# sebcossu/yocto_raytracing

Measured on AMD Instinct MI355X. Metric: Mrays/sec + ms/frame, instance10000 1920×1080×64spp, 1/2/4/8 MI355X, higher is better.
Workload: dtype f32; 1 GPU; instance10000 1920x1080 8x8 spp, amb 0.1, one frame per step; scene=instance10000, width=1920, height=1080, spp=64, parallelism=single GPU, algorithm=wavefront

## Files before the change

yocto_raytracing_amd/csrc/wavefront.hip:

```cpp
#include <hip/hip_runtime.h>

#include <algorithm>
#include <cstdio>
#include <cstdlib>
#include <cstring>
#include <stdexcept>

#include "packet_trace.h"
#include "trace_common.h"
#include "yrt_render.h"

namespace yrt {
namespace {

constexpr int WF_BLOCK = 256;
#ifndef YRT_PRIMARY_BLOCK
#define YRT_PRIMARY_BLOCK 64
#endif
#ifndef YRT_SHADOW_BLOCK
#define YRT_SHADOW_BLOCK 64
#endif
template <bool PACKET>
constexpr int shadow_block() { return PACKET ? YRT_SHADOW_BLOCK : WF_BLOCK; }
#ifndef YRT_TRACE_WAVES
// ... 41 lines not shown
        const float* rays;
    };
    int capacity;
    int nlevels;
    int need_v;
    int bundles;
    f4* pbox;
    int* lcount;
    int* lskip;
    f4* lists;
    f4* slists;
    int cam_lists;
    int* ccount;
    int* cskip;
    f4* clist;
    unsigned long long* lstats;
};

#ifndef YRT_LEVEL_SEGMENTS
#define YRT_LEVEL_SEGMENTS 8
#endif
constexpr int level_segments = YRT_LEVEL_SEGMENTS;
static_assert(2048 % level_segments == 0, "segment bound (run()) assumes level_segments | 2048");
constexpr int count_stride = 32;
__device__ __forceinline__ int* seg_counter(int* count, int level, int g) {
    return count + (level * level_segments + g) * count_stride;
}

struct chunk_args {
    long long pix0;
    int npix;
    int spp;
    int tiles_x;
};

__device__ __forceinline__ bool pixel_of(const dev_render_args& A, int tiles_x, long long p, int& lx, int& ly,
                                         int& i, int& j) {
    long long t = p / (TILE * TILE);
    int w = (int)(p % (TILE * TILE));
    lx = (int)(t % tiles_x) * TILE + (w % TILE);
    ly = (int)(t / tiles_x) * TILE + (w / TILE);
    if (lx >= A.tile_w || ly >= A.tile_h) return false;
    i = A.x0 + lx;
    int b = ly / A.band, r = ly % A.band;
    j = A.y0 + (b * A.band_stride + A.band_offset) * A.band + r;
    return i < A.width && j < A.height;
}

__device__ __forceinline__ void flush(unsigned long long* counters, int idx, unsigned long long v) {
    unsigned long long s = wave_sum(v);
    if ((threadIdx.x & 63) == 0 && s) atomicAdd(counter_line(counters) + idx, s);
}

template <int N, int BS = WF_BLOCK>
__device__ __forceinline__ void flush_block(unsigned long long* counters, const int (&idx)[N],
                                            const unsigned long long (&v)[N]) {
    __shared__ unsigned long long part[BS / 64][N];
    const int w = threadIdx.x >> 6;
#pragma unroll
    for (int k = 0; k < N; k++) {
        const unsigned long long s = wave_sum(v[k]);
        if ((threadIdx.x & 63) == 0) part[w][k] = s;
    }
    __syncthreads();
    if (threadIdx.x < N) {
        unsigned long long t = 0;
#pragma unroll
        for (int q = 0; q < BS / 64; q++) t += part[q][threadIdx.x];
        const unsigned b = (blockIdx.z * gridDim.y + blockIdx.y) * gridDim.x + blockIdx.x;
        if (t) atomicAdd(counters + (size_t)(b % cnt_slots) * cnt_count + idx[threadIdx.x], t);
    }
}

__device__ __forceinline__ void flush_work(unsigned long long* counters, const work_counts& wc) {
    flush(counters, cnt_box_tests, wc.box);
    flush(counters, cnt_inst_entries, wc.inst);
    flush(counters, cnt_prim_tests, wc.prim);
    flush(counters, cnt_shaded_hits, wc.hits);
    flush(counters, cnt_tex_lookups, wc.tex);
    flush(counters, cnt_wave_node_visits, wc.wnode);
    flush(counters, cnt_wave_prim_visits, wc.wprim);
}

typedef float gvec4 __attribute__((ext_vector_type(4)));
#ifndef YRT_NT_STREAMS
#define YRT_NT_STREAMS 1
#endif
#ifndef YRT_R5_VCONST
#define YRT_R5_VCONST 1
#endif
template <int IMM>
__device__ __forceinline__ float vconst() {
    if (!YRT_R5_VCONST) return __int_as_float(IMM);
    float r;
    asm volatile("v_mov_b32 %0, %1" : "=v"(r) : "n"(IMM));
    return r;
}
__device__ __forceinline__ void gstore(f4* p, int idx, float x, float y, float z, float w) {
    auto* q = (__attribute__((address_space(1))) gvec4*)p + idx;
    if (YRT_NT_STREAMS)
        __builtin_nontemporal_store(gvec4{x, y, z, w}, q);
    else
        *q = gvec4{x, y, z, w};
}
__device__ __forceinline__ void gstore(float* p, int idx, float x) {
    auto* q = (__attribute__((address_space(1))) float*)p + idx;
    if (YRT_NT_STREAMS)
        __builtin_nontemporal_store(x, q);
    else
        *q = x;
}
__device__ __forceinline__ float4 ld4s(const f4* p) {
    if (YRT_NT_STREAMS) {
        const gvec4 v = __builtin_nontemporal_load((const __attribute__((address_space(1))) gvec4*)p);
        return make_float4(v.x, v.y, v.z, v.w);
    }
    return ld4(p);
}
__device__ __forceinline__ float lds1(const float* p) {
    if (YRT_NT_STREAMS) return __builtin_nontemporal_load((const __attribute__((address_space(1))) float*)p);
    return *p;
}
__device__ __forceinline__ unsigned char ldb(const unsigned char* p) {
    if (YRT_NT_STREAMS) return __builtin_nontemporal_load((const __attribute__((address_space(1))) unsigned char*)p);
// ... 1255 lines not shown
        elo = lo, ehi = hi;
    }
    const unsigned long long km = ballot(keep);
    if (keep) {
        f4* out = B.clist + ((size_t)t * camera_list_max + __popcll(km & below)) * 2;
        out[0] = {elo.x, elo.y, elo.z, elo.w};
        out[1] = {ehi.x, ehi.y, ehi.z, ehi.w};
    }
    nf = __popcll(km);
    nskip = (int)wave_sum((unsigned long long)nskip);
    if (lane == 0) B.ccount[t] = nf, B.cskip[t] = nskip;
    YRT_LT_STAMP(lt3);
    YRT_LT_WRITE(0, t, lt1 - lt0, lt2 - lt1, lt3 - lt2, (unsigned long long)nrounds << 32 | (unsigned)nf);
}

__global__ __launch_bounds__(256) void k_list_stats(wf_buffers B, int ntiles, int nlists) {
    __shared__ unsigned long long part[list_sums][256 / 64];
    unsigned long long v[list_sums] = {};
    const int stride = gridDim.x * 256;
    if (B.cam_lists)
        for (int i = blockIdx.x * 256 + (int)threadIdx.x; i < ntiles; i += stride) {
            const int n = B.ccount[i];
            v[0] += n < 0 ? camera_list_max + 1 : n, v[1]++, v[4] += (unsigned)B.cskip[i];
        }
    if (B.bundles)
        for (int i = blockIdx.x * 256 + (int)threadIdx.x; i < nlists; i += stride) {
            const int n = B.lcount[i];
            v[2] += n < 0 ? bundle_max + 1 : n, v[3]++, v[5] += (unsigned)B.lskip[i];
        }
    for (int q = 0; q < list_sums; q++) {
        const unsigned long long t = wave_sum(v[q]);
        if ((threadIdx.x & 63) == 0) part[q][threadIdx.x >> 6] = t;
    }
    __syncthreads();
    if (threadIdx.x < list_sums) {
        const unsigned long long t = part[threadIdx.x][0] + part[threadIdx.x][1] + part[threadIdx.x][2] + part[threadIdx.x][3];
        if (t) atomicAdd(B.lstats + threadIdx.x, t);
    }
}

#ifndef YRT_SHADOW_PERSIST_MIN_ITEMS
#define YRT_SHADOW_PERSIST_MIN_ITEMS 262144
#endif
#ifndef YRT_SHADOW_ITEM_LIGHTS
#define YRT_SHADOW_ITEM_LIGHTS 1
#endif
#ifndef YRT_SHADOW_ITEM_RUN
#define YRT_SHADOW_ITEM_RUN 48
#endif
#ifndef YRT_SHADOW_LDS_RECORDS
#define YRT_SHADOW_LDS_RECORDS 85
#endif

template <int LDSN>
__global__ __launch_bounds__(SP_BLOCK, YRT_SHADOW_WAVES) void k_shadow_persist(dev_scene_view S, int nsamp,
                                                                                int nx, wf_buffers B,
                                                                                unsigned long long* counters,
                                                                                float4 cam4) {
    const vec3f cam_o = xyz(cam4);
    constexpr int WPB = SP_BLOCK / 64;
    constexpr unsigned C = (YRT_SHADOW_ITEM_LIGHTS && LDSN == 0) ? YRT_SHADOW_ITEM_RUN : YRT_SHADOW_LIGHT_MINOR;
    __shared__ float4 lds_nodes[LDSN > 0 ? LDSN * 8 : 1];
    if constexpr (LDSN > 0) {
        const int nrec = LDSN * 8;
        const float4* src = reinterpret_cast<const float4*>(S.wnodes);
        for (int i = threadIdx.x; i < nrec; i += SP_BLOCK) lds_nodes[i] = src[i];
        __syncthreads();
    }
    const int nl = S.nlights;
    constexpr bool IL = YRT_SHADOW_ITEM_LIGHTS && LDSN == 0;
    const unsigned n_items = IL ? (unsigned)nx : (unsigned)nx * (unsigned)nl;
    const unsigned lane = threadIdx.x & 63;
    const unsigned xcd = blockIdx.x % 8u;
    unsigned rays = 0;
    unsigned culled_l = 0;
    constexpr unsigned CS = YRT_SHADOW_BLOCK_CHUNK;
    __shared__ chunk_ring ring;
    const unsigned head = head_items<C, CS>(n_items);
    chunk_ring_init<CS>(ring, B.queue + xcd, B.queue + 8, head / 8u);
#ifdef YRT_TAIL_STATS
    const unsigned long long tail_t0 = __builtin_amdgcn_s_memrealtime();
    unsigned tail_items = 0;
#endif
    for (;;) {
        const unsigned q = chunk_ring_next<CS>(ring, B.queue + xcd, lane, B.queue + 8, head / 8u);
        const unsigned it = split_item<C>(q, xcd, n_items, head);
        if (it >= n_items) break;
#ifdef YRT_TAIL_STATS
        tail_items++;
#endif
        const int bx = IL ? (int)it : (int)(it / (unsigned)nl);
        for (int lq = 0; lq < (IL ? nl : 1); lq++) {
        const int li = IL ? lq : (int)(it % (unsigned)nl);
        float4 lrec[6];
        ld_records_at<6>(S.lights, (unsigned)(6 * li), lrec);
        const frame3f lf = {xyz(lrec[0]), xyz(lrec[1]), xyz(lrec[2]), xyz(lrec[3])};
        const vec3f lp0 = xyz(lrec[4]);
        const int idx = bx * 64 + (int)lane;
        bool valid = false;
        int info = -1;
        float r = 1.0f;
        float4 s1 = {0, 0, 0, 0};
        ray3 sr = {{0, 0, 0}, {0, 0, 1}, 0.01f, 1.0f};
        if (idx < nsamp) {
            float4 s0 = IL ? ld4(B.surf0 + idx) : ld4s(B.surf0 + idx);
            if (YRT_SHADOW_CULL && !YRT_HIT16) s1 = IL ? ld4(B.surf1 + idx) : ld4s(B.surf1 + idx);
            info = sample_state(s0);
            if (info >= 0) {
                const vec3f p = YRT_HIT16 ? hit16_surface(S, s0).p : xyz(s0);
                vec3f tp = transform_point(lf, lp0 - p);
                vec3f l;
                normalize_len(tp, l, r);
                sr = {p, l, 0.01f, r - 0.01f};
                valid = true;
            }
        }
        rays += (unsigned)__popcll(ballot(valid));
        const bool zero_term =
            YRT_SHADOW_CULL && !YRT_HIT16 && light_term_zero(info, xyz(s1), sr.o, cam_o, sr.d, r, xyz(lrec[5]));
        const unsigned long long culled = ballot(zero_term);
        culled_l += zero_term ? 1u : 0u;
        const bool all_culled = YRT_SHADOW_CULL && !YRT_HIT16 && culled == ballot(valid);
        bool occ;
        int lc = -1;
        if (YRT_SHADOW_BUNDLES && LDSN == 0 && B.bundles) {
            const int gl = (bx / bundle_g) * nl + li;
            lc = __builtin_amdgcn_readfirstlane(B.lcount[gl]);
        }
        const f4* tbase = S.wnodes;
        uint32_t troot = (uint32_t)S.wtop_root;
        if (lc > 0) {
            tbase = B.lists;
            troot = (uint32_t)(((bx / bundle_g) * nl + li) * bundle_recs * wide_record_bytes);
        }
        occ = all_culled ? true
                         : lc == 0 ? ((culled >> lane) & 1ull) != 0
                                   : packet_occluded_wide2<LDSN, true>(S, sr, valid, lds_nodes, tbase, troot, culled);
        if (valid) stb(B.occl + (size_t)li * B.capacity + idx, occ ? 1 : 0);
        }
    }
#ifdef YRT_TAIL_STATS
    tail_record(1, tail_t0, tail_items);
#endif
    const unsigned long long mine = lane == 0 ? (unsigned long long)rays : 0ull;
    flush_block<2, SP_BLOCK>(counters, {cnt_shadow_rays, cnt_shadow_culled}, {mine, (unsigned long long)culled_l});
}

#ifndef YRT_SHADE_WAVES
#define YRT_SHADE_WAVES 7
#endif
#ifndef YRT_SHADE_LDS_SRGB
#define YRT_SHADE_LDS_SRGB 1
#endif
#ifndef YRT_FOLD_PREFETCH
#define YRT_FOLD_PREFETCH 0
#endif
#ifndef YRT_SHADE_LEVEL_WAVES
#define YRT_SHADE_LEVEL_WAVES 5
#endif
template <bool COUNT, bool FUSE, int SB, bool OCC4, bool RAYS>
__device__ __forceinline__ void shade_samples(dev_scene_view S, dev_render_args A, int level, int nsamp_level0,
                                              int max_depth, wf_buffers B, unsigned long long* counters, chunk_args C,
                                              float4* __restrict__ out) {
    __shared__ float4 fused_rad[FUSE ? SB : 1];
    __shared__ int cmp_count[SB / 64], cmp_base[SB / 64];
    __shared__ float srgb_lds[YRT_SHADE_LDS_SRGB ? 256 : 1];
    const float* lut = YRT_SHADE_LDS_SRGB ? srgb_lds : S.srgb;
    if (YRT_SHADE_LDS_SRGB && S.ntextures > 0) {
        for (int q = (int)threadIdx.x; q < 256; q += SB) srgb_lds[q] = S.srgb[q];
        __syncthreads();
    }
    work_counts wc;
    unsigned long long truncated = 0;
    const vec3f amb = {A.amb[0], A.amb[1], A.amb[2]};
    const vec3f cam_o = {A.cam.ox, A.cam.oy, A.cam.oz};
    const int stride = gridDim.x * SB;
    const int gout = (int)(blockIdx.x % (unsigned)level_segments);
    const int nseg = FUSE ? 1 : level ? level_segments : 1;
    for (int g = 0; g < nseg; g++) {
    const int n = (!FUSE && level) ? *seg_counter(B.count, level, g) : nsamp_level0;
    const int nround = (n + stride - 1) / stride;
    for (int round = 0; round < nround; round++) {
        const int j = round * stride + blockIdx.x * SB + threadIdx.x;
        const int idx = FUSE ? j : g * B.seg + j;
        bool spawn = false;
        vec3f p = {0, 0, 0}, dr = {0, 0, 0}, rec_d = {0, 0, 0}, rec_la = {0, 0, 0};
        int rec_mat = 0;
        if (j < n) {
            float4 s0 = ld4s(B.surf0 + idx);
            uint32_t occ_bits = 0;
            if constexpr (OCC4) {
#pragma unroll
                for (int q = 0; q < 4; q++) {
                    const int lq = q < S.nlights ? q : 0;
                    const uint32_t ob = ldb(B.occl + (size_t)lq * B.capacity + idx);
                    occ_bits |= (q < S.nlights && ob != 0u) ? 1u << q : 0u;
                }
            }
            const int info = sample_state(s0);
            vec3f R = {0, 0, 0};
            bool write_r = info != -2;
            float4 ro4 = (!FUSE && level) ? ld4(B.ray_o(level) + idx) : make_float4(cam_o.x, cam_o.y, cam_o.z, 0.0f);
            if constexpr (RAYS && !FUSE) {
                if (!level) {
                    const vec3f o = ray_origin(B, idx);
                    ro4 = make_float4(o.x, o.y, o.z, 0.0f);
                }
            }
            float4 pd = {0, 0, 0, 0}, pla = {0, 0, 0, 0}, pkr = {0, 0, 0, 0};
            if (YRT_FOLD_PREFETCH && !FUSE && level) {
                const int parent = ibits(ro4.w);
                pd = ld4(B.rec0(level - 1) + parent), pla = ld4(B.rec1(level - 1) + parent);
                pkr = ld4(S.mats + 4 * ibits(pd.w) + 2);
            }
            if (info >= 0) {
                vec3f nrm;
                vec2f uv;
                int mat, kind;
                if (YRT_HIT16) {
                    const surface sf = hit16_surface(S, s0);
                    p = sf.p, nrm = sf.n, uv = sf.uv, mat = sf.mat, kind = sf.kind;
                } else {
                    const float4 s1 = ld4s(B.surf1 + idx);
                    p = xyz(s0), nrm = xyz(s1), uv = {s1.w, (!YRT_SKIP_UNUSED_V || B.need_v) ? lds1(B.surfv + idx) : 0.0f};
                    mat = info_mat(info), kind = info & 3;
                }
                const vec3f ro = xyz(ro4);
                float4 m0, m1, m2, m3;
                {
                    m0 = ld4(S.mats + 4 * mat), m1 = ld4(S.mats + 4 * mat + 1);
                    m2 = ld4(S.mats + 4 * mat + 2), m3 = ld4(S.mats + 4 * mat + 3);
                }
                const vec3f kd0 = xyz(m0), ks0 = xyz(m1), kr = xyz(m2);
                const float ns = m0.w;
                const int kd_txt = ibits(m1.w), ks_txt = ibits(m2.w);
                const bool reflective = ibits(m3.w) & mat_reflective;
                vec3f la = amb * kd0;
                vec3f tkd = {1, 1, 1}, tks = {1, 1, 1};
                if (kd_txt >= 0) {
                    tkd = eval_texture<COUNT>(S, kd_txt, uv, wc, lut);
                    la = la * tkd;
                }
                if (ks_txt >= 0) tks = eval_texture<COUNT>(S, ks_txt, uv, wc, lut);
                vec3f c = {0.0f, 0.0f, 0.0f};
                vec3f v;
                float vlen;
                normalize_len(ro - p, v, vlen);
                for (int li = 0; li < S.nlights; li++) {
                    if (OCC4 ? ((occ_bits >> li) & 1u) != 0u : ldb(B.occl + (size_t)li * B.capacity + idx) != 0) continue;
                    const f4* lr = S.lights + 6 * li;
                    float4 lrec[6];
                    ld_scalar<6>(lr, lrec);
                    frame3f lf = {xyz(lrec[0]), xyz(lrec[1]), xyz(lrec[2]), xyz(lrec[3])};
                    vec3f lp0 = xyz(lrec[4]), ke = xyz(lrec[5]);
                    vec3f tp = transform_point(lf, lp0 - p);
                    vec3f l, h;
                    float r, hlen;
                    normalize_len(tp, l, r);
                    normalize_len(v + l, h, hlen);
                    vec3f kd = kd0, ks = ks0;
                    if (kd_txt >= 0) kd = kd * tkd;
                    if (ks_txt >= 0) ks = ks * tks;
                    const vec3f ker = div3(ke, r * r);
                    vec3f ld = kd * ker;
                    vec3f ls = ks * ker;
                    if (kind == kind_lines) {
                        float prodnl = dot(nrm, l);
                        float prodnh = dot(nrm, h);
                        if (prodnl < 0.0f) prodnl *= -1;
                        if (prodnh < 0.0f) prodnh *= -1;
                        float sinnl = __builtin_sqrtf(1.0f - prodnl);
                        float sinnh = __builtin_sqrtf(1.0f - prodnh);
                        ld = ld * sinnl;
                        ls = ls * spec_pow(sinnh, ns, ls);
                    } else {
                        ld = ld * smax(0.0f, dot(nrm, l));
                        ls = ls * spec_pow(smax(0.0f, dot(nrm, h)), ns, ls);
                    }
                    c = c + (ld + ls);
                }
                if (!reflective) {
                    R = c + la;
                } else if (FUSE || level + 1 >= max_depth || level + 1 >= B.nlevels) {
                    truncated++;
                    vec3f t = {0.0f * kr.x, 0.0f * kr.y, 0.0f * kr.z};
                    R = (c + t) + la;
                } else {
                    spawn = true;
                    dr = (nrm * 2.0f * dot(nrm, v)) - v;
                    rec_d = c;
                    rec_la = la;
                    rec_mat = mat;
                    write_r = false;
                }
                if (COUNT) wc.hits++;
            }
            if (FUSE) {
                fused_rad[threadIdx.x] = make_float4(R.x, R.y, R.z, 1.0f);
            } else if (write_r) {
                vec3f col = R;
                int lev = level, node = idx;
                while (lev > 0) {
                    const bool pre = YRT_FOLD_PREFETCH && lev == level;
                    const int parent = pre ? ibits(ro4.w) : ibits(B.ray_o(lev)[node].w);
                    const float4 d = pre ? pd : ld4(B.rec0(lev - 1) + parent);
                    const float4 la = pre ? pla : ld4(B.rec1(lev - 1) + parent);
                    const float4 kr = pre ? pkr : ld4(S.mats + 4 * ibits(d.w) + 2);
                    vec3f cc = {d.x, d.y, d.z};
                    cc = cc + vec3f{col.x * kr.x, col.y * kr.y, col.z * kr.z};
                    cc = cc + xyz(la);
                    col = cc, node = parent, lev--;
                }
                B.rad[node] = {col.x, col.y, col.z, 1.0f};
            }
        }
        if constexpr (FUSE) continue;
        const unsigned long long mask = __ballot(spawn);
        const int w = threadIdx.x >> 6, lane = threadIdx.x & 63;
        if (spawn) {
            B.rec0(level)[idx] = {rec_d.x, rec_d.y, rec_d.z, __int_as_float(rec_mat)};
            B.rec1(level)[idx] = {rec_la.x, rec_la.y, rec_la.z, 0};
        }
        if (lane == 0) cmp_count[w] = __popcll(mask);
        __syncthreads();
        if (threadIdx.x == 0) {
            int tot = 0;
            for (int q = 0; q < SB / 64; q++) tot += cmp_count[q];
            int acc = tot ? atomicAdd(seg_counter(B.count, level + 1, gout), tot) : 0;
            for (int q = 0; q < SB / 64; q++) cmp_base[q] = acc, acc += cmp_count[q];
        }
        __syncthreads();
        if (spawn) {
            const int slot = gout * B.seg + cmp_base[w] + __popcll(mask & ((1ull << lane) - 1));
            B.ray_o(level + 1)[slot] = {p.x, p.y, p.z, __int_as_float(idx)};
            B.ray_d(level + 1)[slot] = {dr.x, dr.y, dr.z, 0};
        }
    }
    }
    if (FUSE) {
        __syncthreads();
        const int ppb = SB / C.spp;
        for (int t = (int)threadIdx.x; t < 3 * ppb; t += SB) {
            const int px = t / 3, comp = t - 3 * px;
            const int pl = (int)(blockIdx.x * SB / C.spp) + px;
            int lx, ly, i, j;
            const bool valid = pl < C.npix && pixel_of(A, C.tiles_x, C.pix0 + pl, lx, ly, i, j);
            if (pl < C.npix && lx < A.tile_w && ly < A.tile_h) {
                float v = 0.0f;
                if (valid) {
                    const float* r = reinterpret_cast<const float*>(fused_rad + px * C.spp) + comp;
                    float acc = 0.0f;
                    for (int q = 0; q < C.spp; q++) acc = acc + r[4 * q];
                    v = acc / float(C.spp);
                }
                float* o = reinterpret_cast<float*>(out + (size_t)ly * A.out_stride + lx);
                o[comp] = v;
                if (comp == 0) o[3] = valid ? 1.0f : 0.0f;
            }
        }
    }
    flush(counters, cnt_depth_truncated, truncated);
    if (COUNT) flush_work(counters, wc);
}

template <bool COUNT, bool FUSE, int SB = WF_BLOCK, bool OCC4 = false>
__global__ __launch_bounds__(SB, FUSE ? YRT_SHADE_WAVES : YRT_SHADE_LEVEL_WAVES) void k_shade(dev_scene_view S, dev_render_args A, int level, int nsamp_level0,
                                                    int max_depth, wf_buffers B, unsigned long long* counters,
                                                    chunk_args C, float4* __restrict__ out) {
    shade_samples<COUNT, FUSE, SB, OCC4, false>(S, A, level, nsamp_level0, max_depth, B, counters, C, out);
}

template <bool OCC4>
__global__ __launch_bounds__(WF_BLOCK, YRT_SHADE_LEVEL_WAVES) void k_rays_shade(dev_scene_view S, float3 amb3, int level,
                                                                                int nsamp_level0, int max_depth,
                                                                                wf_buffers B,
                                                                                unsigned long long* counters) {
    dev_render_args A = {};
    A.amb[0] = amb3.x, A.amb[1] = amb3.y, A.amb[2] = amb3.z;
    const chunk_args C = {0, nsamp_level0, 1, 1};
    shade_samples<false, false, WF_BLOCK, OCC4, true>(S, A, level, nsamp_level0, max_depth, B, counters, C, nullptr);
}

constexpr int AQ = 8;
__global__ __launch_bounds__(WF_BLOCK) void k_accumulate(dev_render_args A, chunk_args C, wf_buffers B,
                                                         float4* __restrict__ out) {
    __shared__ float4 stage[WF_BLOCK / 64][64 * (AQ + 1)];
    const int w = threadIdx.x >> 6, lane = threadIdx.x & 63;
    const int pl0 = blockIdx.x * WF_BLOCK + w * 64;
    const int np = max(0, min(64, C.npix - pl0));
    float4* S = stage[w];
    const f4* base = B.rad + (size_t)pl0 * C.spp;
    vec4f acc = {0, 0, 0, 0};
    for (int q0 = 0; q0 < C.spp; q0 += AQ) {
        const int qn = min(AQ, C.spp - q0);
        for (int e = lane; e < np * qn; e += 64) {
            const int px = e / qn, q = e % qn;
            S[px * (AQ + 1) + q] = ld4(base + (size_t)px * C.spp + q0 + q);
        }
        __syncthreads();
        if (lane < np)
            for (int q = 0; q < qn; q++) {
                const float4 c = S[lane * (AQ + 1) + q];
                acc = {acc.x + c.x, acc.y + c.y, acc.z + c.z, acc.w + 1.0f};
            }
        __syncthreads();
    }
    if (lane >= np) return;
    const int pl = pl0 + lane;
    int lx, ly, i, j;
    const bool valid = pixel_of(A, C.tiles_x, C.pix0 + pl, lx, ly, i, j);
    if (lx >= A.tile_w || ly >= A.tile_h) return;
    const float d = float(C.spp);
    out[(size_t)ly * A.out_stride + lx] =
        valid ? make_float4(acc.x / d, acc.y / d, acc.z / d, 1.0f) : make_float4(0.0f, 0.0f, 0.0f, 0.0f);
}

constexpr int pass_planes = pass_count + 1;
struct pass_buffers {
    unsigned mask;
    float4* out[pass_planes];
    f4* smp[pass_count];
};

constexpr int shade_pass_waves = 6;
template <bool FUSE, int SB = WF_BLOCK, bool OCC4 = false>
__global__ __launch_bounds__(SB, FUSE ? shade_pass_waves : YRT_SHADE_LEVEL_WAVES) void k_shade_passes(
    dev_scene_view S, dev_render_args A, int level, int nsamp_level0, int max_depth, wf_buffers B, pass_buffers P,
    unsigned long long* counters, chunk_args C) {
    constexpr int ROW = SB + 1;
    __shared__ float fused[FUSE ? pass_planes * 3 * ROW : 1];
    __shared__ int cmp_count[SB / 64], cmp_base[SB / 64];
    __shared__ float srgb_lds[YRT_SHADE_LDS_SRGB ? 256 : 1];
    const float* lut = YRT_SHADE_LDS_SRGB ? srgb_lds : S.srgb;
    if (YRT_SHADE_LDS_SRGB && S.ntextures > 0) {
// ... 353 lines not shown
        if (e != hipSuccess) return e;
        ds.work_bytes = need;
    }
    wf_buffers B = carve(ds.work, cap, spp, ds.nlights, nlevels);
    B.trel = ds.trel;
    B.seg = seg;
    B.need_v = ds.view.ntextures > 0;
    pass_buffers P = {};
    if (passes) {
        P = *passes;
        char* at = (char*)ds.work + workspace_bytes(cap, spp, ds.nlights, nlevels);
        for (int k = 0; k < pass_count && smp_planes; k++)
            if (P.mask >> k & 1) P.smp[k] = (f4*)at, at += align_up(16 * (size_t)pix_per_chunk * spp);
    }
    bool list_stats = false;
    ds.last_camera_lists = ds.last_bundles = false;
    if (!ds.list_stats_host) {
        hipError_t e =
            hipHostMalloc((void**)&ds.list_stats_host, list_sums * sizeof(unsigned long long), hipHostMallocDefault);
        if (e != hipSuccess) return e;
        memset(ds.list_stats_host, 0, list_sums * sizeof(unsigned long long));
    }
    if (!ds.list_stats_ev) {
        hipError_t e = hipEventCreateWithFlags(&ds.list_stats_ev, hipEventDisableTiming);
        if (e != hipSuccess) return e;
    }
    if (nlevels > 1 && !ds.level_count_host) {
        hipError_t e = hipHostMalloc((void**)&ds.level_count_host, sizeof(int) * level_segments * count_stride,
                                     hipHostMallocDefault);
        if (e != hipSuccess) return e;
    }
    if (nlevels > 1 && !ds.level_count_ev) {
        hipError_t e = hipEventCreateWithFlags(&ds.level_count_ev, hipEventDisableTiming);
        if (e != hipSuccess) return e;
    }
    phase_timer& T = ds.timer;
    const bool stage = ds.lds_staging != 0 && !COUNT && PACKET;
    ds.last_lds_staging = 0;
    const float4 cam4 = make_float4(A.cam.ox, A.cam.oy, A.cam.oz, 0.0f);
    const int stride_grid = 2048;
    if (npix_total == 0 && counters) {
        hipError_t e = hipMemsetAsync(counters, 0, (size_t)cnt_slots * cnt_count * sizeof(unsigned long long), stream);
        if (e != hipSuccess) return e;
    }
    for (long long pix0 = 0; pix0 < npix_total; pix0 += pix_per_chunk) {
        chunk_args C = {pix0, (int)std::min<long long>(pix_per_chunk, npix_total - pix0), spp, tiles_x};
        const int nsamp = C.npix * spp;
        const int grid = (nsamp + WF_BLOCK - 1) / WF_BLOCK;
        constexpr int TB = shadow_block<PACKET>();
        const int tgrid = (nsamp + TB - 1) / TB;
        const bool shadow_persist = !COUNT && PACKET && ds.wide_ok && TB == 64 && ds.nlights > 0 &&
                                    ((long long)tgrid * ds.nlights >= YRT_SHADOW_PERSIST_MIN_ITEMS ||
                                     ds.lists_mode == 1 || stage);
        const bool bundles_possible = YRT_SHADOW_BUNDLES && !stage && shadow_persist &&
                                      bundle_lights(ds.nlights) > 0 && ds.view.nwtop >= YRT_BUNDLE_MIN_TOP;
        const bool cam_lists_possible = YRT_CAMERA_LISTS && YRT_PRIMARY_REL && !stage && !COUNT && PACKET && ds.wide_ok &&
                                        ds.view.nwtop >= YRT_BUNDLE_MIN_TOP;
        const bool lists = ds.lists_mode == 1 || (ds.lists_mode == 0 && spp >= YRT_LISTS_MIN_SPP);
        B.cam_lists = cam_lists_possible && lists;
        B.bundles = bundles_possible && lists;
        ds.last_camera_lists |= B.cam_lists != 0, ds.last_bundles |= B.bundles != 0;
        const bool zero_lstats = (B.cam_lists || B.bundles) && !list_stats;
        list_stats |= zero_lstats;
        int t = T.begin(phase_lists, stream);
        {
            const int nrec = (PACKET && pix0 == 0) ? (int)ds.ntnodes * 2 * spine_len : 0;
            const int count_ints = nlevels > 1 ? (int)(count_bytes(nlevels) / sizeof(int)) : 0;
            const int counter_words = pix0 == 0 && counters ? cnt_slots * cnt_count : 0;
            const int work = std::max(std::max(nrec, count_ints), std::max(counter_words, 32));
            const int nb = std::min((work + WF_BLOCK - 1) / WF_BLOCK, 1024);
            hipLaunchKernelGGL(k_chunk_setup, dim3(nb), dim3(WF_BLOCK), 0, stream, nrec ? ds.view.tpair : nullptr,
                               nrec, A.cam.ox, A.cam.oy, A.cam.oz, ds.trel, B.queue,
                               zero_lstats ? B.lstats : nullptr, B.count, count_ints, counters, counter_words);
        }
        if (B.cam_lists) {
            const int nt = C.npix / (TILE * TILE);
            hipLaunchKernelGGL(k_camera_lists, dim3((nt + 3) / 4), dim3(256), 0, stream, ds.view, A, C, B);
        }
        T.end(t, stream);
        t = T.begin(phase_primary, stream);
        bool persist = false;
        if constexpr (!COUNT && PACKET) {
            persist = ((long long)nsamp + 63) / 64 >= (long long)YRT_PRIMARY_PERSIST_MIN_ITEMS;
            if (persist) {
                const int nb = ds.num_cus * (YRT_PRIMARY_WAVES * 4 * 64 / YRT_PRIMARY_SP_BLOCK);
                if (B.cam_lists)
                    hipLaunchKernelGGL((k_primary_persist<SE, 0, true>), dim3(nb), dim3(YRT_PRIMARY_SP_BLOCK), 0,
                                       stream, ds.view, A, C, B, counters);
                else if (stage && YRT_PRIMARY_REL) {
                    hipLaunchKernelGGL((k_primary_persist<SE, YRT_PRIMARY_LDS_RECORDS, false>), dim3(nb),
                                       dim3(YRT_PRIMARY_SP_BLOCK), 0, stream, ds.view, A, C, B, counters);
                    ds.last_lds_staging |= 1;
                } else
                    hipLaunchKernelGGL((k_primary_persist<SE, 0, false>), dim3(nb), dim3(YRT_PRIMARY_SP_BLOCK), 0,
                                       stream, ds.view, A, C, B, counters);
            }
        }
        if (!persist) {
            const dim3 pg((nsamp + YRT_PRIMARY_BLOCK - 1) / YRT_PRIMARY_BLOCK);
            if (B.cam_lists)
                hipLaunchKernelGGL((k_primary<COUNT, PACKET, SE, true>), pg, dim3(YRT_PRIMARY_BLOCK), 0, stream, ds.view,
                                   A, C, B, counters);
            else
                hipLaunchKernelGGL((k_primary<COUNT, PACKET, SE, false>), pg, dim3(YRT_PRIMARY_BLOCK), 0, stream,
                                   ds.view, A, C, B, counters);
        }
        T.end(t, stream);
        for (int level = 0; level < nlevels; level++) {
            if (level > 0) {
                t = T.begin(phase_bounce, stream);
                hipLaunchKernelGGL((k_bounce<COUNT, PACKET, SE>), dim3(stride_grid), dim3(WF_BLOCK), 0, stream, ds.view,
                                   level, B, counters);
                T.end(t, stream);
                hipError_t e = hipEventSynchronize(ds.level_count_ev);
                if (e != hipSuccess) return e;
                bool any = false;
                for (int g = 0; g < level_segments; g++) any |= ds.level_count_host[g * count_stride] != 0;
                if (!any) break;
            }
            if (ds.nlights > 0) {
                dim3 sg(level ? stride_grid * WF_BLOCK / TB : tgrid, ds.nlights);
                if (level == 0 && shadow_persist && B.bundles) {
                    t = T.begin(phase_lists, stream);
                    if (YRT_BUNDLE_FUSED && YRT_BUNDLE_SUPER && bundle_g * super_bundles <= 256) {
                        const long long ns = (long long)super_count(nsamp) * ds.nlights;
                        hipLaunchKernelGGL(k_bundle_lists<true>, dim3((unsigned)ns), dim3(256), 0, stream, ds.view, B,
                                           tgrid);
                    } else {
                        if (YRT_BUNDLE_SUPER) {
                            const long long ns = (long long)super_count(nsamp) * ds.nlights;
                            hipLaunchKernelGGL(k_bundle_super, dim3((unsigned)((ns + 3) / 4)), dim3(256), 0, stream,
                                               ds.view, B, tgrid);
                        }
                        const long long nw = (long long)bundle_count(nsamp) * ds.nlights;
                        hipLaunchKernelGGL(k_bundle_lists<false>, dim3((unsigned)((nw + 3) / 4)), dim3(256), 0, stream,
                                           ds.view, B, tgrid);
                    }
                    T.end(t, stream);
                }
                t = T.begin(phase_shadow, stream);
                if (level == 0 && shadow_persist) {
                    const int nb = ds.num_cus * (YRT_SHADOW_WAVES * 4 * 64 / SP_BLOCK);
                    constexpr int L = YRT_SHADOW_LDS_RECORDS;
                    if (stage && L > 0 && ds.view.nwtop >= L) {
                        hipLaunchKernelGGL((k_shadow_persist<L>), dim3(nb), dim3(SP_BLOCK), 0, stream, ds.view,
                                           nsamp, tgrid, B, counters, cam4);
                        ds.last_lds_staging |= 2;
                    } else
                        hipLaunchKernelGGL((k_shadow_persist<0>), dim3(nb), dim3(SP_BLOCK), 0, stream, ds.view,
                                           nsamp, tgrid, B, counters, cam4);
                } else if (!COUNT && PACKET && ds.wide_ok)
                    hipLaunchKernelGGL((k_shadow<COUNT, PACKET, SE, true>), sg, dim3(TB), 0,
                                       stream, ds.view, level, nsamp, B, counters, cam4);
                else
                    hipLaunchKernelGGL((k_shadow<COUNT, PACKET, SE, false>), sg, dim3(TB), 0,
                                       stream, ds.view, level, nsamp, B, counters, cam4);
                T.end(t, stream);
            }
            t = T.begin(phase_shade, stream);
            const bool occ4 = ds.nlights <= 4;
#define YRT_SHADE_LAUNCH(FU, SBV, GRID)                                                                          \
    do {                                                                                                        \
        if (occ4)                                                                                               \
            hipLaunchKernelGGL((k_shade<COUNT, FU, SBV, true>), GRID, dim3(SBV), 0, stream, ds.view, A, level, nsamp, \
                               A.max_depth, B, counters, C, out);                                               \
        else                                                                                                    \
            hipLaunchKernelGGL((k_shade<COUNT, FU, SBV, false>), GRID, dim3(SBV), 0, stream, ds.view, A, level,      \
                               nsamp, A.max_depth, B, counters, C, out);                                        \
    } while (0)
#define YRT_SHADE_PASSES_LAUNCH(FU, GRID)                                                                          \
    do {                                                                                                          \
        if (occ4)                                                                                                 \
            hipLaunchKernelGGL((k_shade_passes<FU, WF_BLOCK, true>), GRID, dim3(WF_BLOCK), 0, stream, ds.view, A, level, \
                               nsamp, A.max_depth, B, P, counters, C);                                            \
        else                                                                                                      \
            hipLaunchKernelGGL((k_shade_passes<FU, WF_BLOCK, false>), GRID, dim3(WF_BLOCK), 0, stream, ds.view, A,  \
                               level, nsamp, A.max_depth, B, P, counters, C);                                     \
    } while (0)
            if (passes) {
                if constexpr (!COUNT) {
                    if (fuse)
                        YRT_SHADE_PASSES_LAUNCH(true, dim3(grid));
                    else
                        YRT_SHADE_PASSES_LAUNCH(false, dim3(level ? stride_grid : grid));
                }
            } else if (fuse) {
                YRT_SHADE_LAUNCH(true, WF_BLOCK, dim3(grid));
            } else {
                YRT_SHADE_LAUNCH(false, WF_BLOCK, dim3(level ? stride_grid : grid));
            }
#undef YRT_SHADE_PASSES_LAUNCH
#undef YRT_SHADE_LAUNCH
            T.end(t, stream);
            if (level + 1 < nlevels) {
                hipError_t e = hipMemcpyAsync(ds.level_count_host,
                                              B.count + (size_t)(level + 1) * level_segments * count_stride,
                                              sizeof(int) * level_segments * count_stride, hipMemcpyDeviceToHost,
                                              stream);
                if (e == hipSuccess) e = hipEventRecord(ds.level_count_ev, stream);
                if (e != hipSuccess) return e;
            }
        }
        if (!fuse) {
            t = T.begin(phase_accumulate, stream);
            if (passes)
                hipLaunchKernelGGL(k_accumulate_passes, dim3((C.npix + WF_BLOCK - 1) / WF_BLOCK, pass_planes),
                                   dim3(WF_BLOCK), 0, stream, A, C, B, P);
            else
                hipLaunchKernelGGL(k_accumulate, dim3((C.npix + WF_BLOCK - 1) / WF_BLOCK), dim3(WF_BLOCK), 0, stream, A,
                                   C, B, out);
            T.end(t, stream);
// ... 260 lines not shown
```

Baseline: 30040 Mrays/s.

## Fuse shadow tracing and shading into one persistent kernel for single-level renders

Result: faster. 30610 Mrays/s, median of 6 (+1.9%).

```diff
diff --git a/yocto_raytracing_amd/csrc/wavefront.hip b/yocto_raytracing_amd/csrc/wavefront.hip
--- a/yocto_raytracing_amd/csrc/wavefront.hip
+++ b/yocto_raytracing_amd/csrc/wavefront.hip
@@ -117,24 +117,29 @@
     if ((threadIdx.x & 63) == 0 && s) atomicAdd(counter_line(counters) + idx, s);
 }
 
+template <int N, int BS, class F>
+__device__ __forceinline__ void flush_block_at(unsigned long long* counters, const unsigned long long (&v)[N],
+                                               unsigned tid, F index_of) {
+    __shared__ unsigned long long part[BS / 64][N];
+    const int w = tid >> 6;
+#pragma unroll
+    for (int k = 0; k < N; k++) {
+        const unsigned long long s = wave_sum(v[k]);
+        if ((tid & 63) == 0) part[w][k] = s;
+    }
+    __syncthreads();
+    if (tid < N) {
+        unsigned long long t = 0;
+#pragma unroll
+        for (int q = 0; q < BS / 64; q++) t += part[q][tid];
+        const unsigned b = (blockIdx.z * gridDim.y + blockIdx.y) * gridDim.x + blockIdx.x;
+        if (t) atomicAdd(counters + (size_t)(b % cnt_slots) * cnt_count + index_of(tid), t);
+    }
+}
 template <int N, int BS = WF_BLOCK>
 __device__ __forceinline__ void flush_block(unsigned long long* counters, const int (&idx)[N],
                                             const unsigned long long (&v)[N]) {
-    __shared__ unsigned long long part[BS / 64][N];
-    const int w = threadIdx.x >> 6;
-#pragma unroll
-    for (int k = 0; k < N; k++) {
-        const unsigned long long s = wave_sum(v[k]);
-        if ((threadIdx.x & 63) == 0) part[w][k] = s;
-    }
-    __syncthreads();
-    if (threadIdx.x < N) {
-        unsigned long long t = 0;
-#pragma unroll
-        for (int q = 0; q < BS / 64; q++) t += part[q][threadIdx.x];
-        const unsigned b = (blockIdx.z * gridDim.y + blockIdx.y) * gridDim.x + blockIdx.x;
-        if (t) atomicAdd(counters + (size_t)(b % cnt_slots) * cnt_count + idx[threadIdx.x], t);
-    }
+    flush_block_at<N, BS>(counters, v, threadIdx.x, [&](unsigned k) { return idx[k]; });
 }
 
 __device__ __forceinline__ void flush_work(unsigned long long* counters, const work_counts& wc) {
@@ -1496,6 +1501,56 @@
 #define YRT_SHADOW_LDS_RECORDS 85
 #endif
 
+template <int LDSN, bool IL, bool WCULL = false>
+__device__ __forceinline__ bool shadow_item_light(const dev_scene_view& S, const wf_buffers& B, int nsamp, int bx,
+                                                  int li, int nl, unsigned lane, const vec3f& cam_o,
+                                                  const float4* lds_nodes, unsigned& rays, unsigned& culled_n,
+                                                  bool& valid) {
+    float4 lrec[6];
+    ld_records_at<6>(S.lights, (unsigned)(6 * li), lrec);
+    const frame3f lf = {xyz(lrec[0]), xyz(lrec[1]), xyz(lrec[2]), xyz(lrec[3])};
+    const vec3f lp0 = xyz(lrec[4]);
+    const int idx = bx * 64 + (int)lane;
+    valid = false;
+    int info = -1;
+    float r = 1.0f;
+    float4 s1 = {0, 0, 0, 0};
+    ray3 sr = {{0, 0, 0}, {0, 0, 1}, 0.01f, 1.0f};
+    if (idx < nsamp) {
+        float4 s0 = IL ? ld4(B.surf0 + idx) : ld4s(B.surf0 + idx);
+        if (YRT_SHADOW_CULL && !YRT_HIT16) s1 = IL ? ld4(B.surf1 + idx) : ld4s(B.surf1 + idx);
+        info = sample_state(s0);
+        if (info >= 0) {
+            const vec3f p = YRT_HIT16 ? hit16_surface(S, s0).p : xyz(s0);
+            vec3f tp = transform_point(lf, lp0 - p);
+            vec3f l;
+            normalize_len(tp, l, r);
+            sr = {p, l, 0.01f, r - 0.01f};
+            valid = true;
+        }
+    }
+    rays += (unsigned)__popcll(ballot(valid));
+    const bool zero_term =
+        YRT_SHADOW_CULL && !YRT_HIT16 && light_term_zero(info, xyz(s1), sr.o, cam_o, sr.d, r, xyz(lrec[5]));
+    const unsigned long long culled = ballot(zero_term);
+    culled_n += WCULL ? (unsigned)__popcll(culled) : zero_term ? 1u : 0u;
+    const bool all_culled = YRT_SHADOW_CULL && !YRT_HIT16 && culled == ballot(valid);
+    int lc = -1;
+    if (YRT_SHADOW_BUNDLES && LDSN == 0 && B.bundles) {
+        const int gl = (bx / bundle_g) * nl + li;
+        lc = __builtin_amdgcn_readfirstlane(B.lcount[gl]);
+    }
+    const f4* tbase = S.wnodes;
+    uint32_t troot = (uint32_t)S.wtop_root;
+    if (lc > 0) {
+        tbase = B.lists;
+        troot = (uint32_t)(((bx / bundle_g) * nl + li) * bundle_recs * wide_record_bytes);
+    }
+    return all_culled ? true
+                     : lc == 0 ? ((culled >> lane) & 1ull) != 0
+                               : packet_occluded_wide2<LDSN, true>(S, sr, valid, lds_nodes, tbase, troot, culled);
+}
+
 template <int LDSN>
 __global__ __launch_bounds__(SP_BLOCK, YRT_SHADOW_WAVES) void k_shadow_persist(dev_scene_view S, int nsamp,
                                                                                 int nx, wf_buffers B,
@@ -1602,6 +1657,136 @@
 #ifndef YRT_SHADE_LEVEL_WAVES
 #define YRT_SHADE_LEVEL_WAVES 5
 #endif
+__device__ __forceinline__ vec3f amb_of(const vec3f& a) { return a; }
+__device__ __forceinline__ vec3f amb_of(const float* a) { return {a[0], a[1], a[2]}; }
+template <bool COUNT, bool FUSE, bool OCC4, bool LATE = false, class AMB = vec3f>
+__device__ __forceinline__ void shade_hit(const dev_scene_view& S, const wf_buffers& B, int idx, int info,
+                                          const float4& s0, const float4& ro4, uint32_t occ_bits, int level,
+                                          int max_depth, const AMB& amb, const float* lut, work_counts& wc,
+                                          unsigned long long& truncated, vec3f& R, vec3f& p, bool& spawn, vec3f& dr,
+                                          vec3f& rec_d, vec3f& rec_la, int& rec_mat, bool& write_r) {
+    vec3f nrm;
+    vec2f uv;
+    int mat, kind;
+    if (YRT_HIT16) {
+        const surface sf = hit16_surface(S, s0);
+        p = sf.p, nrm = sf.n, uv = sf.uv, mat = sf.mat, kind = sf.kind;
+    } else {
+        const float4 s1 = ld4s(B.surf1 + idx);
+        p = xyz(s0), nrm = xyz(s1), uv = {s1.w, (!YRT_SKIP_UNUSED_V || B.need_v) ? lds1(B.surfv + idx) : 0.0f};
+        mat = info_mat(info), kind = info & 3;
+    }
+    const vec3f ro = xyz(ro4);
+    float4 m0, m1, m2, m3;
+    {
+        m0 = ld4(S.mats + 4 * mat), m1 = ld4(S.mats + 4 * mat + 1);
+        m2 = ld4(S.mats + 4 * mat + 2), m3 = ld4(S.mats + 4 * mat + 3);
+    }
+    const vec3f kd0 = xyz(m0), ks0 = xyz(m1);
+    vec3f kr = xyz(m2);
+    const float ns = m0.w;
+    const int kd_txt = ibits(m1.w), ks_txt = ibits(m2.w);
+    bool reflective = !LATE && (ibits(m3.w) & mat_reflective);
+    vec3f la = {0, 0, 0};
+    if (!LATE) la = amb_of(amb) * kd0;
+    vec3f tkd = {1, 1, 1}, tks = {1, 1, 1};
+    if (kd_txt >= 0) {
+        tkd = eval_texture<COUNT>(S, kd_txt, uv, wc, lut);
+        if (!LATE) la = la * tkd;
+    }
+    if (ks_txt >= 0) tks = eval_texture<COUNT>(S, ks_txt, uv, wc, lut);
+    vec3f c = {0.0f, 0.0f, 0.0f};
+    vec3f v;
+    float vlen;
+    normalize_len(ro - p, v, vlen);
+    for (int li = 0; li < S.nlights; li++) {
+        if (OCC4 ? ((occ_bits >> li) & 1u) != 0u : ldb(B.occl + (size_t)li * B.capacity + idx) != 0) continue;
+        const f4* lr = S.lights + 6 * li;
+        float4 lrec[6];
+        ld_scalar<6>(lr, lrec);
+        frame3f lf = {xyz(lrec[0]), xyz(lrec[1]), xyz(lrec[2]), xyz(lrec[3])};
+        vec3f lp0 = xyz(lrec[4]), ke = xyz(lrec[5]);
+        vec3f tp = transform_point(lf, lp0 - p);
+        vec3f l, h;
+        float r, hlen;
+        normalize_len(tp, l, r);
+        normalize_len(v + l, h, hlen);
+        vec3f kd = kd0, ks = ks0;
+        if (kd_txt >= 0) kd = kd * tkd;
+        if (ks_txt >= 0) ks = ks * tks;
+        const vec3f ker = div3(ke, r * r);
+        vec3f ld = kd * ker;
+        vec3f ls = ks * ker;
+        if (kind == kind_lines) {
+            float prodnl = dot(nrm, l);
+            float prodnh = dot(nrm, h);
+            if (prodnl < 0.0f) prodnl *= -1;
+            if (prodnh < 0.0f) prodnh *= -1;
+            float sinnl = __builtin_sqrtf(1.0f - prodnl);
+            float sinnh = __builtin_sqrtf(1.0f - prodnh);
+            ld = ld * sinnl;
+            ls = ls * spec_pow(sinnh, ns, ls);
+        } else {
+            ld = ld * smax(0.0f, dot(nrm, l));
+            ls = ls * spec_pow(smax(0.0f, dot(nrm, h)), ns, ls);
+        }
+        c = c + (ld + ls);
+    }
+    if (LATE) {
+        la = amb_of(amb) * kd0;
+        if (kd_txt >= 0) la = la * tkd;
+        int matl = info_mat(info);
+        asm volatile("" : "+v"(matl));
+        const f4* ml = S.mats + 4 * matl;
+        reflective = ibits(ld4(ml + 3).w) & mat_reflective;
+        if (reflective) kr = xyz(ld4(ml + 2));
+    }
+    if (!reflective) {
+        R = c + la;
+    } else if (FUSE || level + 1 >= max_depth || level + 1 >= B.nlevels) {
+        truncated++;
+        vec3f t = {0.0f * kr.x, 0.0f * kr.y, 0.0f * kr.z};
+        R = (c + t) + la;
+    } else {
+        spawn = true;
+        dr = (nrm * 2.0f * dot(nrm, v)) - v;
+        rec_d = c;
+        rec_la = la;
+        rec_mat = mat;
+        write_r = false;
+    }
+    if (COUNT) wc.hits++;
+}
+
+template <int STRIDE, int SPP = 0>
+__device__ __forceinline__ void sum_pixels(const dev_render_args& A, const chunk_args& C, float4* __restrict__ out,
+                                           const float4* rad, int pl0, int ppb, int t0) {
+    for (int t = t0; t < 3 * ppb; t += STRIDE) {
+        const int px = t / 3, comp = t - 3 * px;
+        const int pl = pl0 + px;
+        int lx, ly, i, j;
+        const bool valid = pl < C.npix && pixel_of(A, C.tiles_x, C.pix0 + pl, lx, ly, i, j);
+        if (pl < C.npix && lx < A.tile_w && ly < A.tile_h) {
+            float v = 0.0f;
+            if (valid) {
+                const int spp = SPP ? SPP : C.spp;
+                const float* r = reinterpret_cast<const float*>(rad + px * spp) + comp;
+                float acc = 0.0f;
+                if constexpr (SPP > 0) {
+#pragma unroll
+                    for (int q = 0; q < SPP; q++) acc = acc + r[4 * q];
+                } else {
+                    for (int q = 0; q < spp; q++) acc = acc + r[4 * q];
+                }
+                v = acc / float(spp);
+            }
+            float* o = reinterpret_cast<float*>(out + (size_t)ly * A.out_stride + lx);
+            o[comp] = v;
+            if (comp == 0) o[3] = valid ? 1.0f : 0.0f;
+        }
+    }
+}
+
 template <bool COUNT, bool FUSE, int SB, bool OCC4, bool RAYS>
 __device__ __forceinline__ void shade_samples(dev_scene_view S, dev_render_args A, int level, int nsamp_level0,
                                               int max_depth, wf_buffers B, unsigned long long* counters, chunk_args C,
@@ -1658,86 +1843,8 @@
                 pkr = ld4(S.mats + 4 * ibits(pd.w) + 2);
             }
             if (info >= 0) {
-                vec3f nrm;
-                vec2f uv;
-                int mat, kind;
-                if (YRT_HIT16) {
-                    const surface sf = hit16_surface(S, s0);
-                    p = sf.p, nrm = sf.n, uv = sf.uv, mat = sf.mat, kind = sf.kind;
-                } else {
-                    const float4 s1 = ld4s(B.surf1 + idx);
-                    p = xyz(s0), nrm = xyz(s1), uv = {s1.w, (!YRT_SKIP_UNUSED_V || B.need_v) ? lds1(B.surfv + idx) : 0.0f};
-                    mat = info_mat(info), kind = info & 3;
-                }
-                const vec3f ro = xyz(ro4);
-                float4 m0, m1, m2, m3;
-                {
-                    m0 = ld4(S.mats + 4 * mat), m1 = ld4(S.mats + 4 * mat + 1);
-                    m2 = ld4(S.mats + 4 * mat + 2), m3 = ld4(S.mats + 4 * mat + 3);
-                }
-                const vec3f kd0 = xyz(m0), ks0 = xyz(m1), kr = xyz(m2);
-                const float ns = m0.w;
-                const int kd_txt = ibits(m1.w), ks_txt = ibits(m2.w);
-                const bool reflective = ibits(m3.w) & mat_reflective;
-                vec3f la = amb * kd0;
-                vec3f tkd = {1, 1, 1}, tks = {1, 1, 1};
-                if (kd_txt >= 0) {
-                    tkd = eval_texture<COUNT>(S, kd_txt, uv, wc, lut);
-                    la = la * tkd;
-                }
-                if (ks_txt >= 0) tks = eval_texture<COUNT>(S, ks_txt, uv, wc, lut);
-                vec3f c = {0.0f, 0.0f, 0.0f};
-                vec3f v;
-                float vlen;
-                normalize_len(ro - p, v, vlen);
-                for (int li = 0; li < S.nlights; li++) {
-                    if (OCC4 ? ((occ_bits >> li) & 1u) != 0u : ldb(B.occl + (size_t)li * B.capacity + idx) != 0) continue;
-                    const f4* lr = S.lights + 6 * li;
-                    float4 lrec[6];
-                    ld_scalar<6>(lr, lrec);
-                    frame3f lf = {xyz(lrec[0]), xyz(lrec[1]), xyz(lrec[2]), xyz(lrec[3])};
-                    vec3f lp0 = xyz(lrec[4]), ke = xyz(lrec[5]);
-                    vec3f tp = transform_point(lf, lp0 - p);
-                    vec3f l, h;
-                    float r, hlen;
-                    normalize_len(tp, l, r);
-                    normalize_len(v + l, h, hlen);
-                    vec3f kd = kd0, ks = ks0;
-                    if (kd_txt >= 0) kd = kd * tkd;
-                    if (ks_txt >= 0) ks = ks * tks;
-                    const vec3f ker = div3(ke, r * r);
-                    vec3f ld = kd * ker;
-                    vec3f ls = ks * ker;
-                    if (kind == kind_lines) {
-                        float prodnl = dot(nrm, l);
-                        float prodnh = dot(nrm, h);
-                        if (prodnl < 0.0f) prodnl *= -1;
-                        if (prodnh < 0.0f) prodnh *= -1;
-                        float sinnl = __builtin_sqrtf(1.0f - prodnl);
-                        float sinnh = __builtin_sqrtf(1.0f - prodnh);
-                        ld = ld * sinnl;
-                        ls = ls * spec_pow(sinnh, ns, ls);
-                    } else {
-                        ld = ld * smax(0.0f, dot(nrm, l));
-                        ls = ls * spec_pow(smax(0.0f, dot(nrm, h)), ns, ls);
-                    }
-                    c = c + (ld + ls);
-                }
-                if (!reflective) {
-                    R = c + la;
-                } else if (FUSE || level + 1 >= max_depth || level + 1 >= B.nlevels) {
-                    truncated++;
-                    vec3f t = {0.0f * kr.x, 0.0f * kr.y, 0.0f * kr.z};
-                    R = (c + t) + la;
-                } else {
-                    spawn = true;
-                    dr = (nrm * 2.0f * dot(nrm, v)) - v;
-                    rec_d = c;
-                    rec_la = la;
-                    rec_mat = mat;
-                    write_r = false;
-                }
-                if (COUNT) wc.hits++;
+                shade_hit<COUNT, FUSE, OCC4>(S, B, idx, info, s0, ro4, occ_bits, level, max_depth, amb, lut, wc,
+                                             truncated, R, p, spawn, dr, rec_d, rec_la, rec_mat, write_r);
             }
             if (FUSE) {
                 fused_rad[threadIdx.x] = make_float4(R.x, R.y, R.z, 1.0f);
@@ -1784,24 +1891,7 @@
     if (FUSE) {
         __syncthreads();
         const int ppb = SB / C.spp;
-        for (int t = (int)threadIdx.x; t < 3 * ppb; t += SB) {
-            const int px = t / 3, comp = t - 3 * px;
-            const int pl = (int)(blockIdx.x * SB / C.spp) + px;
-            int lx, ly, i, j;
-            const bool valid = pl < C.npix && pixel_of(A, C.tiles_x, C.pix0 + pl, lx, ly, i, j);
-            if (pl < C.npix && lx < A.tile_w && ly < A.tile_h) {
-                float v = 0.0f;
-                if (valid) {
-                    const float* r = reinterpret_cast<const float*>(fused_rad + px * C.spp) + comp;
-                    float acc = 0.0f;
-                    for (int q = 0; q < C.spp; q++) acc = acc + r[4 * q];
-                    v = acc / float(C.spp);
-                }
-                float* o = reinterpret_cast<float*>(out + (size_t)ly * A.out_stride + lx);
-                o[comp] = v;
-                if (comp == 0) o[3] = valid ? 1.0f : 0.0f;
-            }
-        }
+        sum_pixels<SB>(A, C, out, fused_rad, (int)(blockIdx.x * SB / C.spp), ppb, (int)threadIdx.x);
     }
     flush(counters, cnt_depth_truncated, truncated);
     if (COUNT) flush_work(counters, wc);
@@ -1824,6 +1914,106 @@
     const chunk_args C = {0, nsamp_level0, 1, 1};
     shade_samples<false, false, WF_BLOCK, OCC4, true>(S, A, level, nsamp_level0, max_depth, B, counters, C, nullptr);
 }
+
+#if !defined(YRT_SHADOW_SHADE_FUSE)
+#define YRT_SHADOW_SHADE_FUSE 1
+#endif
+#if (YRT_SHADOW_SHADE_FUSE && YRT_SHADOW_ITEM_LIGHTS && YRT_SHADOW_CULL && !YRT_HIT16)
+#define YRT_SHADOW_SHADE_KERNEL 1
+#else
+#define YRT_SHADOW_SHADE_KERNEL 0
+#endif
+#if (YRT_SHADOW_SHADE_KERNEL)
+__global__ __launch_bounds__(SP_BLOCK, YRT_SHADOW_WAVES) void k_shadow_shade_persist(dev_scene_view S,
+                                                                                      dev_render_args A, int nsamp,
+                                                                                      int nx, wf_buffers B,
+                                                                                      unsigned long long* counters,
+                                                                                      chunk_args C,
+                                                                                      float4* __restrict__ out) {
+    constexpr int WPB = SP_BLOCK / 64;
+    constexpr unsigned RUN = YRT_SHADOW_ITEM_RUN;
+    __shared__ float4 wave_rad[WPB][64];
+    __shared__ unsigned wave_truncated[WPB];
+    __shared__ float srgb_lds[YRT_SHADE_LDS_SRGB ? 256 : 1];
+    __shared__ struct {
+        dev_render_args A;
+        chunk_args C;
+    } args;
+    const float* lut = YRT_SHADE_LDS_SRGB ? srgb_lds : S.srgb;
+    if (YRT_SHADE_LDS_SRGB && S.ntextures > 0)
+        for (int q = (int)threadIdx.x; q < 256; q += SP_BLOCK) srgb_lds[q] = S.srgb[q];
+    if (threadIdx.x == 0) args.A = A, args.C = C;
+    __syncthreads();
+    float cam_x = A.cam.ox, cam_y = A.cam.oy, cam_z = A.cam.oz;
+    asm volatile("" : "+s"(cam_x), "+s"(cam_y), "+s"(cam_z));
+    const vec3f cam_o = {cam_x, cam_y, cam_z};
+    const int nl = S.nlights;
+    __builtin_assume(nl > 0);
+    const unsigned n_items = (unsigned)nx;
+    auto lane_now = []() {
+        unsigned l;
+        asm volatile("v_mbcnt_lo_u32_b32 %0, -1, 0\n\tv_mbcnt_hi_u32_b32 %0, -1, %0" : "=v"(l));
+        return l;
+    };
+    const int w = __builtin_amdgcn_readfirstlane((int)(threadIdx.x >> 6));
+    const unsigned xcd = blockIdx.x % 8u;
+    unsigned rays = 0, culled = 0;
+    if (lane_now() == 0) wave_truncated[w] = 0;
+    constexpr unsigned CS = YRT_SHADOW_BLOCK_CHUNK;
+    __shared__ chunk_ring ring;
+    const unsigned head = head_items<RUN, CS>(n_items);
+    chunk_ring_init<CS>(ring, B.queue + xcd, B.queue + 8, head / 8u);
+    for (;;) {
+        const unsigned q = chunk_ring_next<CS>(ring, B.queue + xcd, lane_now(), B.queue + 8, head / 8u);
+        const unsigned it = split_item<RUN>(q, xcd, n_items, head);
+        if (it >= n_items) break;
+        const int bx = (int)it;
+        uint32_t occ_bits = 0;
+        for (int li = 0; li < nl; li++) {
+            bool valid;
+            const bool occ = shadow_item_light<0, true, true>(S, B, nsamp, bx, li, nl, lane_now(), cam_o, nullptr, rays,
+                                                              culled, valid);
+            occ_bits |= (occ ? 1u : 0u) << li;
+        }
+        const int idx = bx * 64 + (int)lane_now();
+        vec3f R = {0, 0, 0};
+        unsigned long long truncated = 0;
+        if (idx < nsamp) {
+            const float4 s0 = ld4(B.surf0 + idx);
+            const int info = sample_state(s0);
+            if (info >= 0) {
+                const float4 ro4 = make_float4(cam_o.x, cam_o.y, cam_o.z, 0.0f);
+                const float* amb = args.A.amb;
+                work_counts wc;
+                vec3f p = {0, 0, 0}, dr = {0, 0, 0}, rec_d = {0, 0, 0}, rec_la = {0, 0, 0};
+                int rec_mat = 0;
+                bool spawn = false, write_r = true;
+                shade_hit<false, true, true, true>(S, B, idx, info, s0, ro4, occ_bits, 0, 1, amb, lut, wc, truncated, R, p,
+                                             spawn, dr, rec_d, rec_la, rec_mat, write_r);
+            }
+        }
+        const unsigned lane = lane_now();
+        const unsigned ntrunc = (unsigned)__popcll(ballot(truncated != 0));
+        if (ntrunc && lane == 0) wave_truncated[w] += ntrunc;
+        wave_rad[w][lane] = make_float4(R.x, R.y, R.z, 1.0f);
+        asm volatile("s_waitcnt lgkmcnt(0)" ::: "memory");
+        const int spp = __builtin_amdgcn_readfirstlane(args.C.spp);
+        if (spp == 64) {
+            sum_pixels<64, 64>(args.A, args.C, out, wave_rad[w], bx, 1, (int)lane);
+        } else {
+            const int sl = __builtin_ctz((unsigned)spp);
+            sum_pixels<64>(args.A, args.C, out, wave_rad[w], bx << (6 - sl), 64 >> sl, (int)lane);
+        }
+        asm volatile("s_waitcnt lgkmcnt(0)" ::: "memory");
+    }
+    const unsigned lane = lane_now();
+    const unsigned long long first = lane == 0 ? 1ull : 0ull;
+    flush_block_at<3, SP_BLOCK>(
+        counters, {first * rays, first * culled, first * (lane == 0 ? wave_truncated[w] : 0u)},
+        (unsigned)w * 64u + lane,
+        [](unsigned k) { return k == 0 ? cnt_shadow_rays : k == 1 ? cnt_shadow_culled : cnt_depth_truncated; });
+}
+#endif
 
 constexpr int AQ = 8;
 __global__ __launch_bounds__(WF_BLOCK) void k_accumulate(dev_render_args A, chunk_args C, wf_buffers B,
@@ -2283,6 +2473,8 @@
         const bool shadow_persist = !COUNT && PACKET && ds.wide_ok && TB == 64 && ds.nlights > 0 &&
                                     ((long long)tgrid * ds.nlights >= YRT_SHADOW_PERSIST_MIN_ITEMS ||
                                      ds.lists_mode == 1 || stage);
+        const bool shadow_shade = YRT_SHADOW_SHADE_KERNEL && shadow_persist && !stage &&
+                                  nlevels == 1 && !passes && 64 % spp == 0 && ds.nlights <= 32;
         const bool bundles_possible = YRT_SHADOW_BUNDLES && !stage && shadow_persist &&
                                       bundle_lights(ds.nlights) > 0 && ds.view.nwtop >= YRT_BUNDLE_MIN_TOP;
         const bool cam_lists_possible = YRT_CAMERA_LISTS && YRT_PRIMARY_REL && !stage && !COUNT && PACKET && ds.wide_ok &&
@@ -2377,7 +2569,13 @@
                         hipLaunchKernelGGL((k_shadow_persist<L>), dim3(nb), dim3(SP_BLOCK), 0, stream, ds.view,
                                            nsamp, tgrid, B, counters, cam4);
                         ds.last_lds_staging |= 2;
-                    } else
+                    }
+#if (YRT_SHADOW_SHADE_KERNEL)
+                    else if (shadow_shade)
+                        hipLaunchKernelGGL(k_shadow_shade_persist, dim3(nb), dim3(SP_BLOCK), 0, stream, ds.view, A,
+                                           nsamp, tgrid, B, counters, C, out);
+#endif
+                    else
                         hipLaunchKernelGGL((k_shadow_persist<0>), dim3(nb), dim3(SP_BLOCK), 0, stream, ds.view,
                                            nsamp, tgrid, B, counters, cam4);
                 } else if (!COUNT && PACKET && ds.wide_ok)
@@ -2388,6 +2586,7 @@
                                        stream, ds.view, level, nsamp, B, counters, cam4);
                 T.end(t, stream);
             }
+            if (level == 0 && shadow_shade) continue;
             t = T.begin(phase_shade, stream);
             const bool occ4 = ds.nlights <= 4;
 #define YRT_SHADE_LAUNCH(FU, SBV, GRID)                                                                          \
```
